# raulmur/ORB_SLAM

Measured on AMD Instinct MI355X. Metric: frames/s ORB extract+match @640x480, 1000 kp, higher is better.
Workload: dtype u8; 1 GPU; vga: 640x480 grayscale stream, 8 levels, nFeatures 1000, S-blocks frames, extract + Hamming top-2 match vs previous frame (BASELINE.json configs[1] + the frame-to-frame match of the metric); resident_frames_per_gpu=2048, lanes=4, parity_checked_frames=0, parity_mismatches=0, library_build_id=3635dfdd85252d64, lane_placement=2

## Files before the change

orb_slam_amd/csrc/k_fast.hip:

```cpp
#include <algorithm>
#include <type_traits>

#include "orbx_device.h"
#include "orbx_launch.h"
#include "k_blur_strip.h"

namespace orbx {

__device__ __forceinline__ int fast_pair_test(const uint8_t* c, int S, int v, int t) {
    const int x0 = c[3 * S], x1 = c[3 * S + 1], x2 = c[2 * S + 2], x3 = c[S + 3], x4 = c[3], x5 = c[-S + 3], x6 = c[-2 * S + 2], x7 = c[-3 * S + 1];
    const int x8 = c[-3 * S], x9 = c[-3 * S - 1], x10 = c[-2 * S - 2], x11 = c[-S - 3], x12 = c[-3], x13 = c[S - 3], x14 = c[2 * S - 2], x15 = c[3 * S - 1];
    const int a = imax3(imax3(imin(x0, x8), imin(x1, x9), imin(x2, x10)), imax3(imin(x3, x11), imin(x4, x12), imin(x5, x13)), imax(imin(x6, x14), imin(x7, x15)));
    const int bq = imin3(imin3(imax(x0, x8), imax(x1, x9), imax(x2, x10)), imin3(imax(x3, x11), imax(x4, x12), imax(x5, x13)), imin(imax(x6, x14), imax(x7, x15)));
    return (int)(v - a > t) | (int)(bq - v > t);
}

__device__ __forceinline__ int fast_score_raw(const uint8_t* c, int S, int v, int tmin) {
    int x[16];
    x[0] = c[3 * S]; x[1] = c[3 * S + 1]; x[2] = c[2 * S + 2]; x[3] = c[S + 3]; x[4] = c[3]; x[5] = c[-S + 3]; x[6] = c[-2 * S + 2]; x[7] = c[-3 * S + 1];
    x[8] = c[-3 * S]; x[9] = c[-3 * S - 1]; x[10] = c[-2 * S - 2]; x[11] = c[-S - 3]; x[12] = c[-3]; x[13] = c[S - 3]; x[14] = c[2 * S - 2]; x[15] = c[3 * S - 1];
    int hi3[16], lo3[16];
#pragma unroll
    for (int k = 0; k < 16; k++) {
        hi3[k] = imax3(x[k], x[(k + 1) & 15], x[(k + 2) & 15]);
// ... 16 lines not shown
struct FastHdr { int n_hi, n_lo, overflow, pad1; int wsum[8]; int pad2[4]; };
static_assert(sizeof(FastHdr) == 64, "LDS carve");

__device__ __forceinline__ int lane_rank(unsigned long long m) {
    return (int)__builtin_amdgcn_mbcnt_hi((unsigned)(m >> 32), __builtin_amdgcn_mbcnt_lo((unsigned)m, 0u));
}
struct CompassK { uint32_t R, KB, KD; };
__device__ __forceinline__ CompassK compass_consts(int t) {
    CompassK k;
    k.R = (uint32_t)compass_r(t) * 0x01010101u;
    k.KB = (uint32_t)compass_kb(t) * 0x01010101u;
    k.KD = (uint32_t)compass_kd(t) * 0x01010101u;
    return k;
}
__device__ __forceinline__ uint32_t compass4_dev(uint32_t C, uint32_t E, uint32_t W, uint32_t Nn, uint32_t Ss, const CompassK& k) {
    const uint32_t nc = ~C;
    const uint32_t hN = __builtin_amdgcn_lerp(Nn, nc, k.R), hS = __builtin_amdgcn_lerp(Ss, nc, k.R);
    const uint32_t hE = __builtin_amdgcn_lerp(E, nc, k.R), hW = __builtin_amdgcn_lerp(W, nc, k.R);
    const uint32_t br = (__builtin_amdgcn_lerp(hN, k.KB, 0u) | __builtin_amdgcn_lerp(hS, k.KB, 0u)) &
                        (__builtin_amdgcn_lerp(hE, k.KB, 0u) | __builtin_amdgcn_lerp(hW, k.KB, 0u));
    const uint32_t dN = __builtin_amdgcn_lerp(hN, k.KD, 0u), dS = __builtin_amdgcn_lerp(hS, k.KD, 0u);
    const uint32_t dE = __builtin_amdgcn_lerp(hE, k.KD, 0u), dW = __builtin_amdgcn_lerp(hW, k.KD, 0u);
    return (br | ~((dN & dS) | (dE & dW))) & 0x80808080u;
}
__global__ void k_eval_compass(const uint32_t* c, const uint32_t* e, const uint32_t* w, const uint32_t* nn, const uint32_t* ss, uint32_t* out, int n, int t) {
    const int i = blockIdx.x * blockDim.x + threadIdx.x;
    if (i < n) out[i] = compass4_dev(c[i], e[i], w[i], nn[i], ss[i], compass_consts(t));
}
int launch_eval_compass(const uint32_t* c, const uint32_t* e, const uint32_t* w, const uint32_t* nn, const uint32_t* ss, uint32_t* out, int n, int t) {
    hipLaunchKernelGGL(k_eval_compass, dim3((n + 255) / 256), dim3(256), 0, 0, c, e, w, nn, ss, out, n, t);
    return hipGetLastError() == hipSuccess ? ORBX_OK : ORBX_ERR_DEVICE;
}

template <bool ALIGNED, int NT, int PPT, bool GATHER = false>
__device__ __forceinline__ void fast_band_task(const Batch& b, int frame, int item, uint8_t* smem) {
    constexpr int NW = NT / 64;
    static_assert((NW & (NW - 1)) == 0, "wave roles rotate modulo NW");
    constexpr int Q0CAP = fast_q0cap(PPT), Q1CAP = FAST_Q1CAP, Q2CAP = FAST_Q2CAP, Q3CAP = FAST_Q3CAP;
    constexpr int WQ_BYTES = fast_wave_queue_bytes(PPT);
    const DevGeom& g = b.g;
    const BandGeom bg = b.bands[item];
    const int level = bg.level;
    const LevelGeom& L = g.lv[level];
    const int lane = threadIdx.x & 63, wave = ORBX_FAST_ROTATE ? (wave_id() + item) & (NW - 1) : wave_id(), tid = wave * 64 + lane;
    const int cw = bg.x1 - bg.x0 + 1, ch = bg.ey1 - bg.ey0 + 1;
    CellState* cst = b.cstate + (long long)frame * g.nbands_total + item;
    const int hint = b.fallback_hint ? (int)((uint32_t)cst->thr >> 8) : 0;
    if (cw <= 0 || ch <= 0) {
        if (tid == 0) { CellState st; st.n_all = 0; st.n_hi = 0; st.n_lo = 0; st.thr = g.tmin; *cst = st; }
        return;
    }
    const int own_lo = bg.y0 - bg.ey0, own_hi = bg.y1 - bg.ey0;
    const int gxb = (bg.x0 - 3) & ~3;
    const int xoff = (bg.x0 - 3) - gxb;
    const int nd = fast_row_dwords(xoff, cw);
    const int S = nd * 4;
    const int x_first = xoff + 3;
    const int nrows = ch + 6;
    FastHdr* hdr = reinterpret_cast<FastHdr*>(smem);
    unsigned long long* cmask = reinterpret_cast<unsigned long long*>(smem + sizeof(FastHdr));
    uint8_t* wq = smem + sizeof(FastHdr) + g.fast_max_chunks * 8 + wave * WQ_BYTES;
    uint32_t* q0 = reinterpret_cast<uint32_t*>(wq);
    uint16_t* q1 = reinterpret_cast<uint16_t*>(wq + Q0CAP * 4);
    uint16_t* q2 = q1 + Q1CAP;
    uint16_t* q3 = q2 + Q2CAP;
    uint8_t* s_img = smem + sizeof(FastHdr) + g.fast_max_chunks * 8 + NW * WQ_BYTES;
    uint8_t* s_sc = s_img + g.fast_max_img;
    const int q_own_lo = (3 + own_lo) * S, q_own_hi = (3 + own_hi + 1) * S;
    const int nchunks = (q_own_hi - q_own_lo + 63) >> 6;
    long long stride64;
    const uint8_t* src = plain_plane<GATHER>(b, L, level, frame, stride64);
    auto clear_lds = [&]() {
        for (int i = tid; i < ((nrows * S + 15) >> 4); i += NT) reinterpret_cast<uint4*>(s_sc)[i] = make_uint4(0, 0, 0, 0);
        if (tid < (int)(sizeof(FastHdr) / 4)) reinterpret_cast<int*>(hdr)[tid] = 0;
        for (int i = tid; i < nchunks; i += NT) cmask[i] = 0ull;
    };
    if (ALIGNED) {
        typedef const void __attribute__((address_space(1))) * gptr_t;
        typedef void __attribute__((address_space(3))) * lptr_t;
        const uint8_t* src0 = src + (long long)(bg.ey0 - 3) * stride64 + gxb;
        clear_lds();
        {
            const int cpr = nd >> 2, nchunks16 = nrows * cpr;
            const float inv_cpr = bg.inv_cpr;
            for (int q0 = 64 * wave; q0 < nchunks16; q0 += 64 * NW) {
                const int q = q0 + lane;
                int r, c;
                split_px(imin(q, nchunks16 - 1), cpr, inv_cpr, r, c);
                const uint8_t* ga = src0 + (long long)r * stride64 + 16 * c;
                if (q < nchunks16) __builtin_amdgcn_global_load_lds((gptr_t)ga, (lptr_t)(s_img + 16 * q0), 16, 0, 0);
            }
        }
        asm volatile("s_waitcnt vmcnt(0)" ::: "memory");
    } else {
        const int total = nrows * nd;
        const float inv_nd0 = bg.inv_nd;
        const uint8_t* src0 = src + (long long)(bg.ey0 - 3) * stride64 + gxb;
        const int xm = L.w - 1 - gxb;
        for (int i0 = 0; i0 < total; i0 += NT * 8) {
            uint32_t v4[8];
#pragma unroll
            for (int k = 0; k < 8; k++) {
                const int i = i0 + k * NT + tid;
                v4[k] = 0;
                if (i < total) {
                    int r, d;
                    split_px(i, nd, inv_nd0, r, d);
                    const uint8_t* row = src0 + (long long)r * stride64;
                    v4[k] = (uint32_t)row[imin(4 * d, xm)] | (uint32_t)row[imin(4 * d + 1, xm)] << 8 | (uint32_t)row[imin(4 * d + 2, xm)] << 16 |
                            (uint32_t)row[imin(4 * d + 3, xm)] << 24;
                }
            }
            if (i0 == 0) clear_lds();
#pragma unroll
            for (int k = 0; k < 8; k++) {
                const int i = i0 + k * NT + tid;
                if (i < total) reinterpret_cast<uint32_t*>(s_img)[i] = v4[k];
            }
        }
    }
    __syncthreads();

    constexpr int FAST_HINT_RUN = 6;
    int tmin = ORBX_FAST_TWO_PASS ? (hint >= FAST_HINT_RUN && g.fast_th > 7 ? 7 : g.fast_th) : g.tmin;
    const float inv_nd = bg.inv_nd;
    int n0 = 0, n1 = 0, n2 = 0, n3 = 0;

    auto score_vals = [&](bool on, int p) {
        int sc = 0;
        if (on) {
            const uint8_t* c = s_img + p;
            sc = fast_score_raw(c, S, c[0], tmin);
            s_sc[p] = (uint8_t)sc;
        }
        const unsigned long long mk = __ballot(sc != 0);
        if (mk) {
            const int add = __popcll(mk);
            if (n3 + add <= Q3CAP) { if (sc) q3[n3 + lane_rank(mk)] = (uint16_t)p; }
            n3 += add;
        }
    };
    auto score_step = [&](const uint16_t* q, int m) { score_vals(lane < m, lane < m ? (int)q[lane] : 0); };
    auto pair_step = [&](const uint16_t* q, int m) {
        int pass = 0, p = 0;
        if (lane < m) {
            p = q[lane];
            const uint8_t* c = s_img + p;
            pass = fast_pair_test(c, S, c[0], tmin);
        }
        const unsigned long long mk = __ballot(pass);
        if (mk) {
            if (pass) q2[n2 + lane_rank(mk)] = (uint16_t)p;
            n2 += __popcll(mk);
            if (n2 >= 64) { n2 -= 64; score_step(q2 + n2, 64); }
// ... 80 lines not shown
            if (s >= 7) atomicAdd(&hdr->n_lo, 1);
        }
    };
    if (!hdr->overflow) {
        int c_hi = 0, c_lo = 0;
        for (int i0 = 0; i0 < n3; i0 += 64) {
            const int i = i0 + lane;
            int s = 0;
            bool keep = false;
            if (i < n3) {
                const int p = q3[i];
                s = s_sc[p];
                keep = p >= q_own_lo && p < q_own_hi && nms_test(p, s);
            }
            c_hi += __popcll(__ballot(keep && s >= g.fast_th));
            c_lo += __popcll(__ballot(keep && s >= 7));
        }
        if (lane == 0 && (c_hi | c_lo)) { atomicAdd(&hdr->n_hi, c_hi); atomicAdd(&hdr->n_lo, c_lo); }
    } else {
        const int d_lo = q_own_lo >> 2, d_hi = q_own_hi >> 2;
        for (int i = d_lo + tid; i < d_hi; i += NT) {
            uint32_t sc4 = reinterpret_cast<const uint32_t*>(s_sc)[i];
            while (sc4) {
                const int j = (__ffs((int)sc4) - 1) >> 3;
                const int s = (int)((sc4 >> (8 * j)) & 255u);
                sc4 &= ~(255u << (8 * j));
                nms_px(4 * i + j, s);
            }
        }
    }
    __syncthreads();
    if (tmin <= 7 || __builtin_amdgcn_readfirstlane(hdr->n_hi) > 3) break;
    __syncthreads();
    clear_lds();
    tmin = 7;
    K = compass_consts(7);
    n0 = n1 = n2 = n3 = 0;
    __syncthreads();
    }
    Cand* out = b.cand + (long long)frame * g.frame_cands + L.cand_base + bg.cand_off;
    const float inv_S = bg.inv_s;
    int run_base = 0;
    for (int c0 = 0; c0 < nchunks; c0 += NT) {
        const bool busy = c0 + 64 * wave < nchunks;
        unsigned long long m = 0ull;
        int cnt = 0, incl = 0;
        if (busy) {
            if (c0 + tid < nchunks) m = cmask[c0 + tid];
            cnt = __popcll(m);
            incl = wave_scan_inclusive(cnt);
        }
        if (NW > 1) {
            if (lane == 63) hdr->wsum[wave] = incl;
            __syncthreads();
        }
        int run = run_base + incl - cnt, total = NW > 1 ? 0 : __builtin_amdgcn_readlane(incl, 63);
        if (NW > 1 && busy) {
#pragma unroll
            for (int wv = 0; wv < NW; wv++) { const int t = hdr->wsum[wv]; if (wv < wave) run += t; total += t; }
        }
        while (m) {
            const int bit = __ffsll((long long)m) - 1;
            m &= m - 1;
            const int p = q_own_lo + (c0 + tid) * 64 + bit;
            int r, xr;
            split_px(p, S, inv_S, r, xr);
            Cand e;
            e.pos = (uint32_t)(bg.x0 + xr - x_first) | ((uint32_t)(bg.ey0 + r - 3) << 16);
            e.resp = (float)s_sc[p];
            out[run++] = e;
        }
        run_base += total;
        if (NW > 1 && c0 + NT < nchunks) __syncthreads();
    }
    if (tid == 0) {
        CellState st;
        st.n_all = run_base; st.n_hi = hdr->n_hi; st.n_lo = hdr->n_lo;
        st.thr = tmin | ((st.n_hi <= 3 && g.fast_th > 7 ? imin(hint + 1, FAST_HINT_RUN) : 0) << 8);
        *cst = st;
    }
}

template <bool ALIGNED, int NT, int PPT, bool GATHER>
__device__ __forceinline__ void k_fast_cells_body(const Batch& b) {
    extern __shared__ __attribute__((aligned(16))) uint8_t smem[];
    int frame, item;
    if (!frame_item_magic(b, blockIdx.x, (unsigned)b.g.nbands_total, b.g.nbands_magic, frame, item)) return;
    fast_band_task<ALIGNED, NT, PPT, GATHER>(b, frame, item, smem);
}
template <bool ALIGNED, int NT, int PPT>
__global__ __launch_bounds__(NT) void k_fast_cells(Batch b) { k_fast_cells_body<ALIGNED, NT, PPT, false>(b); }
template <bool ALIGNED, int NT, int PPT>
__global__ __launch_bounds__(NT) void k_fast_cells_gather(Batch b) { k_fast_cells_body<ALIGNED, NT, PPT, true>(b); }

template <bool ALIGNED, bool SMALL, bool GATHER>
__device__ __forceinline__ void k_fast_blur_body(const Batch& b) {
    extern __shared__ __attribute__((aligned(16))) uint8_t smem[];
    constexpr FastShape A = SMALL ? FAST_SMALL : FAST_LARGE;
    constexpr int NW = A.threads / 64;
    const DevGeom& g = b.g;
    const int nblur = (g.nbtiles_total_s + NW - 1) / NW;
    const int per_frame = nblur + g.nbands_total;
    const int frame = blockIdx.x / per_frame, item = blockIdx.x - frame * per_frame;
    if (item < nblur) {
        const int t = item * NW + wave_id();
        if (t < g.nbtiles_total_s) blur_strip<ALIGNED, BLUR_ROWS_SMALL, GATHER>(b, frame, t);
    } else fast_band_task<ALIGNED, A.threads, A.ppt, GATHER>(b, frame, item - nblur, smem);
}
template <bool ALIGNED, bool SMALL>
__global__ __launch_bounds__(SMALL ? FAST_SMALL.threads : FAST_LARGE.threads) void k_fast_blur(Batch b) { k_fast_blur_body<ALIGNED, SMALL, false>(b); }
template <bool ALIGNED, bool SMALL>
__global__ __launch_bounds__(SMALL ? FAST_SMALL.threads : FAST_LARGE.threads) void k_fast_blur_gather(Batch b) { k_fast_blur_body<ALIGNED, SMALL, true>(b); }


int launch_fast(const Batch& b, const HostGeom& hg, hipStream_t stream, bool fuse_blur) {
    const DevGeom& g = hg.g;
    const int F = b.nframes;
    const bool aligned = (level0_bits(b) & 3) == 0;
    const size_t lds = (size_t)g.fast_lds_bytes;
    auto launch = [&](auto kern, int threads) -> bool {
        if (lds > 64 * 1024 && hipFuncSetAttribute(reinterpret_cast<const void*>(kern), hipFuncAttributeMaxDynamicSharedMemorySize, (int)lds) != hipSuccess) return false;
        hipLaunchKernelGGL(kern, dim3(frame_item_blocks(b, g.nbands_total)), dim3(threads), lds, stream, b);
        return true;
    };
    constexpr FastShape A = FAST_SMALL, B = FAST_LARGE;
    bool ok;
    if (fuse_blur) {
        const int threads = g.fast_small ? A.threads : B.threads;
        const int per_frame = (g.nbtiles_total_s + threads / 64 - 1) / (threads / 64) + g.nbands_total;
        auto launch2 = [&](auto kern) -> bool {
            if (lds > 64 * 1024 && hipFuncSetAttribute(reinterpret_cast<const void*>(kern), hipFuncAttributeMaxDynamicSharedMemorySize, (int)lds) != hipSuccess) return false;
            hipLaunchKernelGGL(kern, dim3(F * per_frame), dim3(threads), lds, stream, b);
            return true;
        };
        if (b.img_tab) {
            if (g.fast_small) ok = aligned ? launch2(k_fast_blur_gather<true, true>) : launch2(k_fast_blur_gather<false, true>);
            else ok = aligned ? launch2(k_fast_blur_gather<true, false>) : launch2(k_fast_blur_gather<false, false>);
        } else if (g.fast_small) ok = aligned ? launch2(k_fast_blur<true, true>) : launch2(k_fast_blur<false, true>);
        else ok = aligned ? launch2(k_fast_blur<true, false>) : launch2(k_fast_blur<false, false>);
    } else if (b.img_tab) {
        if (g.fast_small) ok = aligned ? launch(k_fast_cells_gather<true, A.threads, A.ppt>, A.threads) : launch(k_fast_cells_gather<false, A.threads, A.ppt>, A.threads);
        else ok = aligned ? launch(k_fast_cells_gather<true, B.threads, B.ppt>, B.threads) : launch(k_fast_cells_gather<false, B.threads, B.ppt>, B.threads);
    } else if (g.fast_small) ok = aligned ? launch(k_fast_cells<true, A.threads, A.ppt>, A.threads) : launch(k_fast_cells<false, A.threads, A.ppt>, A.threads);
    else ok = aligned ? launch(k_fast_cells<true, B.threads, B.ppt>, B.threads) : launch(k_fast_cells<false, B.threads, B.ppt>, B.threads);
    if (!ok) return ORBX_ERR_DEVICE;
    ORBX_LAUNCH_CHECK();
    return ORBX_OK;
}

}
```

orb_slam_amd/csrc/orbx_api.hip:

```cpp
#include <climits>
#include <cstdio>
#include <cstdlib>
#include <cstring>

#include "orbx_internal.h"

namespace orbx {
int launch_eval_math(int kind, const float* in0, const float* in1, float* out0, float* out1, int n);
int launch_eval_compass(const uint32_t* c, const uint32_t* e, const uint32_t* w, const uint32_t* nn, const uint32_t* ss, uint32_t* out, int n, int t);
int launch_eval_blur_window(const uint8_t* win, uint8_t* out, int n, int ties_even, int general);
void stage_timer_collect(StageTimer& t);
int launch_debug_nth(const float* d_resp, int n, int nth, int* d_out);
int launch_ingest(uint8_t* d_dst, const uint8_t* mapped_src, size_t bytes, hipStream_t stream);
}
using namespace orbx;

struct orbx_extractor {
    orbx_params p;
    std::string err;
    int gw = 0, gh = 0;
    HostGeom hg;
    struct __attribute__((visibility("hidden"))) Geom {
        DevBuf cells, cellrecs, bands, tabx, taby, pyr_tab;
        DevBuf pyr, blur, cand, sel, cstate, csel, cbands, level_total, level_count, status, long_cells;
    } geo;
    bool fallback_hint = true;
    DevBuf d_img1;
    PinnedBuf h_img1;
    DevBuf d_out1;
    PinnedBuf h_out1;
    bool zero_copy = true;
    Stream s1;
    int stop_after = -1;
    bool no_xcd_affinity = false;
    int od_min_frames = ORBX_OD_MIN_FRAMES_DEFAULT;
    int blur_on_demand = ORBX_BLUR_ON_DEMAND_DEFAULT;
    StageTimer timer;
    SideStream side;
    Batch last;
    bool have_last = false;
    int ph_done = 0;
    struct PhaseKey {
        const void *img, *kps, *desc, *n, *stream;
        int nframes, w, hgt, cap;
        ptrdiff_t row_stride, frame_stride;
        bool operator==(const PhaseKey& o) const {
            return img == o.img && kps == o.kps && desc == o.desc && n == o.n && stream == o.stream && nframes == o.nframes && w == o.w && hgt == o.hgt &&
                   cap == o.cap && row_stride == o.row_stride && frame_stride == o.frame_stride;
        }
    } ph_key = {};
    static constexpr int TAB_RING = 4;
    DevBuf d_tab;
    PinnedBuf h_tab;
    Event tab_ev[TAB_RING];
    int tab_next = 0;
    std::vector<ImgSrc> last_tab;
// ... 4 lines not shown
        Event up_ev[2], kern_ev[2];
        int next = 0;
    };
    HostUpload hup;
    HostUpload cup;
    DevBuf d_cring;
    PinnedBuf h_cimg1, h_gray1;
    DevBuf d_cimg1;
};

template <typename T>
static int upload(orbx_extractor* h, DevBuf& d, const std::vector<T>& v) {
    HIPCHK(h, d.ensure(std::max<size_t>(v.size(), 1) * sizeof(T)));
    if (!v.empty()) HIPCHK(h, hipMemcpy(d, v.data(), v.size() * sizeof(T), hipMemcpyHostToDevice));
    return ORBX_OK;
}

static int ensure_geometry(orbx_extractor* h, int w, int hgt) {
    if (h->gw == w && h->gh == hgt) return ORBX_OK;
    HIPCHK(h, hipDeviceSynchronize());
    h->geo = {};
    h->gw = h->gh = 0;
    h->have_last = false;
    HostGeom hg;
    int rc = build_geometry(h->p, w, hgt, hg, h->err);
    if (rc != ORBX_OK) return rc;
    h->hg = hg;
    const DevGeom& g = h->hg.g;
    const size_t B = (size_t)h->p.max_batch;
    orbx_extractor::Geom& d = h->geo;
    if ((rc = upload(h, d.cells, h->hg.cells)) != ORBX_OK) return rc;
    if ((rc = upload(h, d.cellrecs, h->hg.cellrecs)) != ORBX_OK) return rc;
    if ((rc = upload(h, d.bands, h->hg.bands)) != ORBX_OK) return rc;
    if ((rc = upload(h, d.tabx, h->hg.tabx)) != ORBX_OK) return rc;
    if ((rc = upload(h, d.taby, h->hg.taby)) != ORBX_OK) return rc;
    if ((rc = upload(h, d.pyr_tab, h->hg.pyr_tab)) != ORBX_OK) return rc;
    HIPCHK(h, d.pyr.ensure(B * g.frame_plane_bytes));
    HIPCHK(h, d.blur.ensure(B * g.frame_plane_bytes));
    HIPCHK(h, d.cand.ensure(B * std::max(g.frame_cands, 1) * sizeof(Cand)));
    HIPCHK(h, d.sel.ensure((B * std::max(g.frame_sel, 1) + 4) * sizeof(Cand)));
    HIPCHK(h, d.cstate.ensure(B * g.nbands_total * sizeof(CellState)));
    HIPCHK(h, hipMemset(d.cstate, 0, B * g.nbands_total * sizeof(CellState)));
    HIPCHK(h, d.csel.ensure(B * g.ncells_total * sizeof(CellSel)));
    HIPCHK(h, d.cbands.ensure(B * g.ncells_total * sizeof(CellBands)));
    HIPCHK(h, hipMemset(d.cbands, 0, B * g.ncells_total * sizeof(CellBands)));
    HIPCHK(h, d.level_total.ensure(B * MAX_LEVELS * sizeof(int32_t)));
    HIPCHK(h, d.level_count.ensure(B * MAX_LEVELS * sizeof(int32_t)));
    HIPCHK(h, hipMemset(d.level_total, 0, B * MAX_LEVELS * sizeof(int32_t)));
    HIPCHK(h, hipMemset(d.level_count, 0, B * MAX_LEVELS * sizeof(int32_t)));
    HIPCHK(h, d.status.ensure(B * sizeof(int32_t)));
    HIPCHK(h, d.long_cells.ensure((B * g.ncells_total + 64) * sizeof(int32_t)));
    HIPCHK(h, hipDeviceSynchronize());
    h->gw = w;
    h->gh = hgt;
    return ORBX_OK;
}

static void fill_batch(orbx_extractor* h, Batch& b) {
    const orbx_extractor::Geom& d = h->geo;
    b.g = h->hg.g; b.cells = d.cells.as<CellGeom>(); b.cellrec = d.cellrecs.as<CellRec>(); b.bands = d.bands.as<BandGeom>(); b.tabx = d.tabx.as<ResizeX>(); b.taby = d.taby.as<ResizeY>();
    b.pyr_tab = d.pyr_tab.as<int>(); b.pyr = d.pyr.as(); b.blur = d.blur.as();
    b.cand = d.cand.as<Cand>(); b.sel = d.sel.as<Cand>(); b.cstate = d.cstate.as<CellState>(); b.csel = d.csel.as<CellSel>(); b.cbands = d.cbands.as<CellBands>();
    b.level_total = d.level_total.as<int32_t>(); b.level_count = d.level_count.as<int32_t>(); b.status = d.status.as<int32_t>();
    b.long_cells = d.long_cells.as<int32_t>();
}

static void group_batch(orbx_extractor* h, Batch& b, int f0, int n, orbx_keypoint* d_kps, uint8_t* d_desc, int32_t* d_n, int cap, int32_t* d_status) {
    memset(&b, 0, sizeof(b));
    fill_batch(h, b);
    b.fallback_hint = h->fallback_hint ? 1 : 0;
    b.nframes = n;
    b.xcd_affinity = (b.nframes >= XCD_AFFINITY_MIN_FRAMES && !h->no_xcd_affinity) ? 1 : 0;
    b.blur_on_demand = h->blur_on_demand;
    b.od_min_frames = h->od_min_frames;
    b.out_kps = d_kps + (size_t)f0 * cap;
    b.out_desc = d_desc + (size_t)f0 * cap * 32;
    b.out_n = d_n + f0;
    b.out_status = d_status ? d_status + f0 : nullptr;
    b.cap = cap;
}

static hipMemoryType host_memory_type(const void* p) {
    hipPointerAttribute_t a;
    if (hipPointerGetAttributes(&a, p) != hipSuccess) {
        (void)hipGetLastError();
        return hipMemoryTypeUnregistered;
    }
    return a.type;
}

static int launch_group(orbx_extractor* h, const Batch& b, hipStream_t stream, int phases = ORBX_PHASE_ALL) {
    const int rc = launch_extract(b, h->hg, stream, h->stop_after, &h->timer, &h->side, phases);
    if (rc != ORBX_OK) { h->err = "kernel launch failed (no gfx950 code object for this device?)"; return rc; }
// ... 807 lines not shown
```

orb_slam_amd/csrc/orbx_geometry.hip:

```cpp
#include <cfloat>
#include <climits>
#include <cmath>
#include <cstdlib>
#include <cstring>

#include "k_resize_strip.h"
#include "orbx_internal.h"

namespace orbx {

static inline int round_even(double v) { return (int)std::lrint(v); }
static inline int floor_int(double v) { int i = (int)v; return i - (i > v); }
static inline int ceil_int(double v) { int i = (int)v; return i + (i < v); }
static inline int16_t sat16(float v) {
    int iv = round_even(v);
    return (int16_t)(iv < SHRT_MIN ? SHRT_MIN : iv > SHRT_MAX ? SHRT_MAX : iv);
}
static inline int align_up(int v, int a) { return (v + a - 1) / a * a; }

StripChoice resize_strip_choice(const HostGeom& hg, int level, long long src_stride, unsigned long long src_bits) {
    StripChoice sc = {0, 0};
    const DevGeom& g = hg.g;
    if (level < 1 || level >= g.nlevels) return sc;
    const LevelGeom& L = g.lv[level];
    const LevelGeom& P = g.lv[level - 1];
    if (!L.rz_window) return sc;
    long long stride = P.stride;
    if (level == 1) {
        stride = src_stride;
        if (((src_bits | (unsigned long long)stride) & 3) != 0 || stride < P.w) return sc;
    }
    const long long readable = rzs_readable(level == 1, stride, P.w);
    if (stride > RZS_LDS_BUDGET) return sc;
    const ResizeY* ty = hg.taby.data() + L.taby_off;
    sc.rows_out = rzs_pick_rows(ty, L.h, stride, readable);
    if (sc.rows_out) sc.lds_bytes = (int)rzs_lds_bytes(ty, L.h, sc.rows_out, stride, readable);
    return sc;
}

static int build_geometry_band(const orbx_params& p, int w, int h, HostGeom& out, std::string& err, const int band_px, const FastShape& shape) {
    const int threads = shape.threads;
    const int nl = p.nlevels;
    if (nl < 1 || nl > MAX_LEVELS) { err = "nlevels out of range [1,16]"; return ORBX_ERR_ARG; }
    if (p.nfeatures < 1) { err = "nfeatures must be >= 1"; return ORBX_ERR_ARG; }
    if (!(p.scale_factor > 1.0f) || p.scale_factor > 2.5f) { err = "scale_factor must be in (1, 2.5]"; return ORBX_ERR_ARG; }
    if (w < 1 || h < 1 || w > 16384 || h > 16384) { err = "image size out of range"; return ORBX_ERR_ARG; }
    if (p.score_type != ORBX_HARRIS_SCORE && p.score_type != ORBX_FAST_SCORE) { err = "score_type"; return ORBX_ERR_ARG; }

    out = HostGeom();
    DevGeom& g = out.g;
    memset(&g, 0, sizeof(g));
    g.nlevels = nl;
    g.score_type = p.score_type;
    g.fp_contract = p.fp_contract ? 1 : 0;
    g.fast_th = std::min(std::max(p.fast_th, 0), 255);
    g.tmin = std::min(g.fast_th, 7);

    const double scaleFactor = (double)p.scale_factor;
    out.scale.assign(nl, 1.f);
    out.inv_scale.assign(nl, 1.f);
    for (int i = 1; i < nl; i++) out.scale[i] = (float)(out.scale[i - 1] * scaleFactor);
    const float invScaleFactor = (float)(1.0f / scaleFactor);
    for (int i = 1; i < nl; i++) out.inv_scale[i] = out.inv_scale[i - 1] * invScaleFactor;
    out.features_per_level.assign(nl, 0);
    {
        const float factor = (float)(1.0 / scaleFactor);
        float per_scale = p.nfeatures * (1 - factor) / (1 - (float)std::pow((double)factor, (double)nl));
        int sum = 0;
        for (int l = 0; l < nl - 1; l++) {
            out.features_per_level[l] = round_even(per_scale);
// ... 88 lines not shown
                const bool skipX = (j == levelCols - 1) && (maxBX + 3 - (c.x0 - 3) <= 0);
                const bool skipY = (i == levelRows - 1) && (maxBY + 3 - (c.y0 - 3) <= 0);
                c.skipped = (skipX || skipY) ? 1 : 0;
                const int cw = std::max(0, c.x1 - c.x0 + 1), ch = std::max(0, c.y1 - c.y0 + 1);
                c.cand_off = cand_off;
                c.band0 = (int)out.bands.size();
                const int nb = std::max(1, (cw * ch + band_px - 1) / band_px);
                const int rb = std::max(1, (ch + nb - 1) / nb);
                c.nbands = 0;
                c.cand_cap = 0;
                for (int k = 0; k < nb; k++) {
                    BandGeom bg;
                    memset(&bg, 0, sizeof(bg));
                    bg.x0 = c.x0; bg.x1 = c.x1;
                    bg.y0 = (int16_t)(c.y0 + k * rb);
                    bg.y1 = (int16_t)std::min<int>(c.y1, bg.y0 + rb - 1);
                    if (k > 0 && bg.y0 > c.y1) break;
                    bg.ey0 = (int16_t)std::max<int>(c.y0, bg.y0 - 1);
                    bg.ey1 = (int16_t)std::min<int>(c.y1, bg.y1 + 1);
                    bg.level = l;
                    const int bh = std::max(0, bg.y1 - bg.y0 + 1);
                    bg.cand_off = cand_off;
                    bg.cand_cap = ((cw + 1) / 2) * ((bh + 1) / 2);
                    if (cw > 0) {
                        const int nd = fast_row_dwords((bg.x0 - 3) & 3, cw);
                        bg.inv_nd = 1.0f / (float)nd;
                        bg.inv_s = 1.0f / (float)(nd * 4);
                        bg.inv_cpr = 1.0f / (float)(nd >> 2);
                    }
                    cand_off += bg.cand_cap;
                    c.cand_cap += bg.cand_cap;
                    c.nbands++;
                    out.bands.push_back(bg);
                }
                out.cells.push_back(c);
            }
        for (int ci = L.cell_base; ci < L.cell_base + L.ncells; ci++) {
            const CellGeom& c = out.cells[ci];
            CellRec r;
            memset(&r, 0, sizeof(r));
            r.level = l; r.nbands = c.nbands; r.skipped = c.skipped; r.band0 = c.band0;
            r.sel_base = sel_base; r.plane_off = L.plane_off; r.stride = L.stride;
            r.cand_off = L.cand_base + c.cand_off;
            for (int k = 0; k < c.nbands && k < CELL_REC_BANDS; k++) r.band_cand[k] = L.cand_base + out.bands[c.band0 + k].cand_off;
            out.cellrecs.push_back(r);
        }
        cell_base += L.ncells;
        cand_base += cand_off;
        L.sel_base = sel_base;
        L.sel_cap = std::min(cand_off, L.ncells * L.nfeat_cell + L.ncells * L.ncells + L.ndesired + 64);
        sel_base += L.sel_cap;
        L.slot_base = slot_base;
        slot_base += L.ndesired;
        L.quad_base = quad_base;
        quad_base += (L.ndesired + 3) / 4;

        L.btiles_x = (L.w + 247) / 248;
        L.btiles_y = (L.h + BLUR_ROWS - 1) / BLUR_ROWS;
        L.btile_base = btile_base;
        btile_base += L.btiles_x * L.btiles_y;
        L.btiles_y_s = (L.h + BLUR_ROWS_SMALL - 1) / BLUR_ROWS_SMALL;
        L.btile_base_s = btile_base_s;
        btile_base_s += L.btiles_x * L.btiles_y_s;
        {
            const int nsteps = (L.h + 31) / 32;
            L.mb_strips = (L.w + 32 * MB_TILES - 1) / (32 * MB_TILES);
// ... 92 lines not shown
                        if (s0 < dk) src = is_x ? (out.tabx[Lk.tabx_off + s0].sx & ~3) : out.taby[Lk.taby_off + s0].sy0;
                        at(k - 1, i, 0) = src;
                    }
                    for (int i = 0; i < n; i++) {
                        const int e0 = std::min(at(k, i, 1), dk - 1);
                        int need = is_x ? out.tabx[Lk.tabx_off + e0].sx1 : out.taby[Lk.taby_off + e0].sy1;
                        need = std::max(need, at(k - 1, i + 1, 0) - 1);
                        if (is_x) need = std::min(need | 3, ds - 1);
                        at(k - 1, i, 1) = std::max(need, at(k - 1, i, 0));
                    }
                    at(k - 1, n, 1) = ds;
                }
                return base;
            };
            pg.xtab = chain(pg.ntx, tile[0], true, out.pyr_tab);
            pg.ytab = chain(pg.nty, tile[1], false, out.pyr_tab);
            int off = 0;
            for (int k = 0; k < pg.depth; k++) {
                int maxw = 4, maxh = 1;
                for (int i = 0; i < pg.ntx; i++) maxw = std::max(maxw, out.pyr_tab[pg.xtab + ((size_t)k * (pg.ntx + 1) + i) * 2 + 1] - out.pyr_tab[pg.xtab + ((size_t)k * (pg.ntx + 1) + i) * 2] + 1);
                for (int i = 0; i < pg.nty; i++) maxh = std::max(maxh, out.pyr_tab[pg.ytab + ((size_t)k * (pg.nty + 1) + i) * 2 + 1] - out.pyr_tab[pg.ytab + ((size_t)k * (pg.nty + 1) + i) * 2] + 1);
                pg.pitch[k] = align_up(maxw, 4) + 4;
                pg.lds_off[k] = off;
                off += align_up(pg.pitch[k] * maxh, 16);
            }
            pg.lds_bytes = off;
            if (off > 64 * 1024) { ok = false; break; }
            g.pyr[g.npyr_groups++] = pg;
            l0 += pg.depth;
        }
        if (!ok) { g.npyr_groups = 0; out.pyr_tab.clear(); }
    }
    {
        int max_px = 0, max_img = 0, max_chunks = 0;
        for (const BandGeom& c : out.bands) {
            const int cw = c.x1 - c.x0 + 1, ch = c.ey1 - c.ey0 + 1;
            if (cw <= 0 || ch <= 0) continue;
            max_px = std::max(max_px, cw * ch);
            if (cw > shape.max_cw) { err = "grid cell wider than " + std::to_string(shape.max_cw) + " pixels"; return ORBX_ERR_CAPACITY; }
            const int nd = fast_row_dwords(3, cw);
            max_img = std::max(max_img, nd * 4 * (ch + 6));
            max_chunks = std::max(max_chunks, (nd * 4 * (c.y1 - c.y0 + 1) + 63) / 64);
        }
        if (max_px > 65535 || max_img > 65536) { err = "grid cell band larger than 64 KiB with its halo"; return ORBX_ERR_CAPACITY; }
        g.fast_max_img = align_up(std::max(max_img, 16), 16);
        g.fast_max_chunks = align_up(max_chunks + 1, 2);
        g.fast_lds_bytes = 64  + g.fast_max_chunks * 8 + (threads / 64) * fast_wave_queue_bytes(shape.ppt) + 2 * g.fast_max_img + 16;
        if (g.fast_lds_bytes > 160 * 1024) { err = "grid cell does not fit the 160 KiB LDS"; return ORBX_ERR_CAPACITY; }
    }
    {
        int max_cell = 1, max_level = 1;
        for (const CellGeom& c : out.cells) max_cell = std::max(max_cell, (int)c.cand_cap);
        for (int l = 0; l < nl; l++) max_level = std::max(max_level, g.lv[l].sel_cap);
        g.sel_lds_entries = std::min(std::max(max_cell, max_level), 2048);
        g.sel_lds_cell = align_up(g.sel_lds_entries * ((int)sizeof(Cand) + 4), 16);
        g.sel_lds_level = g.sel_lds_cell;
        if (g.sel_lds_cell > 160 * 1024 || g.sel_lds_level > 160 * 1024) { err = "keypoint list does not fit the 160 KiB LDS"; return ORBX_ERR_CAPACITY; }
    }
    for (int l = 0; l < MAX_LEVELS; l++) {
        const bool live = l < nl;
        g.cell_bases[l] = live ? g.lv[l].cell_base : INT_MAX;
        g.quad_bases[l] = live ? g.lv[l].quad_base : INT_MAX;
        g.btile_bases[l] = live ? g.lv[l].btile_base : INT_MAX;
        g.btile_bases_s[l] = live ? g.lv[l].btile_base_s : INT_MAX;
        g.mb_bases[l] = live ? g.lv[l].mb_base : INT_MAX;
    }
    g.ncells_total = cell_base;
    g.nbands_total = (int)out.bands.size();
    g.nbands_magic = g.nbands_total > 1 ? (uint32_t)((1ull << 32) / (unsigned)g.nbands_total) + 1u : 0u;
    g.nbtiles_total = btile_base;
    g.nbtiles_total_s = btile_base_s;
    g.nmb_total = mb_base;
    g.nslots = slot_base;
    g.nquads = quad_base;
    g.frame_plane_bytes = align_up(plane_off, 256);
    g.frame_cands = cand_base;
    g.frame_sel = sel_base;
    return ORBX_OK;
// ... 42 lines not shown
```

orb_slam_amd/csrc/orbx_internal.h:

```cpp
#pragma once
#include <hip/hip_runtime.h>
#include <stdint.h>
#include <string>
#include <vector>

#include "orbx.h"
#include "orbx_host.h"

namespace orbx {

constexpr int MAX_LEVELS = 16;
constexpr int EDGE = 16;
constexpr int HALF_PATCH = 15;

struct Cand {
    uint32_t pos;
    float resp;
};

struct ResizeX { int16_t sx, sx1, a0, a1; };
struct ResizeY { int16_t sy0, sy1, b0, b1; };

struct LevelGeom {
    int w, h;
// ... 68 lines not shown
#endif
constexpr int MB_WAVES = ORBX_MB_WAVES;
constexpr int BLUR_ROWS = ORBX_BLUR_ROWS;
constexpr int BLUR_ROWS_SMALL = 8;
constexpr int RZ_ROWS = ORBX_RZ_ROWS;
struct FastShape { int threads, ppt, band_px, max_cw; };
#ifndef ORBX_FS
#define ORBX_FS 256, 1, 8192, 500
#endif
#ifndef ORBX_FL
#define ORBX_FL 256, 2, 7168, 6500
#endif
constexpr FastShape FAST_SMALL = {ORBX_FS};
constexpr FastShape FAST_LARGE = {ORBX_FL};
#ifndef ORBX_FAST_TWO_PASS
#define ORBX_FAST_TWO_PASS 1
#endif
#ifndef ORBX_FAST_ROTATE
#define ORBX_FAST_ROTATE 1
#endif
constexpr int FAST_Q1CAP = 192, FAST_Q2CAP = 128, FAST_Q3CAP = 192;
constexpr int fast_q0cap(int) { return 128; }
constexpr int fast_wave_queue_bytes(int ppt) { return fast_q0cap(ppt) * 4 + FAST_Q1CAP * 2 + FAST_Q2CAP * 2 + FAST_Q3CAP * 2; }
__host__ __device__ constexpr int fast_row_dwords(int xoff, int cw) { return (((xoff + cw + 6 + 3) >> 2) + 3) & ~3; }
struct BandGeom {
    int16_t x0, x1;
    int16_t y0, y1;
    int16_t ey0, ey1;
    int32_t level;
    int32_t cand_off;
    int32_t cand_cap;
    float inv_nd, inv_s, inv_cpr;
};

constexpr int XCD_AFFINITY_MIN_FRAMES = 64;
#ifndef ORBX_PYR_DEPTH
#define ORBX_PYR_DEPTH 4, 4
#endif
constexpr int PYR_MAX_GROUPS = 4, PYR_MAX_DEPTH = 8;
struct PyrGroup {
    int l0, depth;
    int ntx, nty;
    int xtab, ytab;
    int lds_off[PYR_MAX_DEPTH];
    int pitch[PYR_MAX_DEPTH];
    int lds_bytes;
};
#ifndef ORBX_PYR_TILE
#define ORBX_PYR_TILE 16, 16
#endif

constexpr int QUOTA_LDS_PER_CELL = 10;
constexpr int QUOTA_MAX_CELLS = 160 * 1024 / QUOTA_LDS_PER_CELL / 64 * 64;
struct CellState { int32_t n_all, n_hi, n_lo, thr; };
constexpr int CELL_REC_BANDS = 8;
struct alignas(64) CellRec {
    int32_t level, nbands, skipped, band0;
    int32_t sel_base;
    int32_t plane_off, stride;
    int32_t cand_off;
    int32_t band_cand[CELL_REC_BANDS];
};
struct alignas(16) CellSel { int32_t n_all, thr, nretain, out_off; };
struct alignas(32) CellBands { int32_t n[CELL_REC_BANDS]; };
static_assert(sizeof(CellRec) == 64 && sizeof(CellSel) == 16 && sizeof(CellBands) == 32, "one scalar load per record");

// ... 4 lines not shown
    uint32_t nbands_magic;
    int nbtiles_total, nbtiles_total_s;
    int nmb_total;
    int nslots;
    int nquads;
    int quota_cells;
    int score_type, fast_th, tmin;
    int fp_contract;
    int frame_plane_bytes;
    int frame_cands;
    int frame_sel;
    int sel_lds_cell, sel_lds_level, sel_lds_entries;
    int fast_max_img, fast_max_chunks, fast_lds_bytes;
    int fast_threads;
    int fast_small;
    int npyr_groups;
    PyrGroup pyr[PYR_MAX_GROUPS];
    int umax[HALF_PATCH + 1];
    int cell_bases[MAX_LEVELS], quad_bases[MAX_LEVELS], btile_bases[MAX_LEVELS], btile_bases_s[MAX_LEVELS], mb_bases[MAX_LEVELS];
    LevelGeom lv[MAX_LEVELS];
};

struct ImgSrc {
    const uint8_t* data;
    long long row_stride;
};
static_assert(sizeof(ImgSrc) == 16, "one scalar dwordx4 per table entry");

struct Batch {
    DevGeom g;
    const CellGeom* cells;
    const CellRec* cellrec;
    const BandGeom* bands;
    const ResizeX* tabx;
    const ResizeY* taby;
    const int* pyr_tab;
    const uint8_t* img;
    long long img_row_stride, img_frame_stride;
    uint8_t* pyr;
    uint8_t* blur;
    Cand* cand;
    Cand* sel;
    CellState* cstate;
    int fallback_hint;
    CellSel* csel;
    CellBands* cbands;
    int32_t* level_total;
    int32_t* level_count;
    int32_t* status;
    int32_t* long_cells;
    orbx_keypoint* out_kps;
    uint8_t* out_desc;
    int32_t* out_n;
    int32_t* out_status;
    int cap;
    int nframes;
    int xcd_affinity;
    int od_min_frames;
    int blur_on_demand;
    const ImgSrc* img_tab;
    unsigned long long img_tab_bits;
    long long img_tab_min_stride;
    long long img_tab_max_stride;
};

static inline unsigned long long level0_bits(const Batch& b) {
    return b.img_tab ? b.img_tab_bits : ((uintptr_t)b.img | (unsigned long long)b.img_row_stride | (unsigned long long)b.img_frame_stride);
}
static inline long long level0_min_stride(const Batch& b) { return b.img_tab ? b.img_tab_min_stride : b.img_row_stride; }
static inline long long level0_max_stride(const Batch& b) { return b.img_tab ? b.img_tab_max_stride : b.img_row_stride; }

struct ColorArgs {
    const uint8_t* src;
    long long src_row_stride, src_frame_stride;
    const ImgSrc* tab;
    unsigned long long tab_bits;
    uint8_t* dst;
    uint8_t* dst2;
    long long dst_row_stride, dst_frame_stride;
    int w, h;
    int f0;
    int cpr, items;
};
static inline int pix_channels(int fmt) {
    switch (fmt) {
        case ORBX_PIX_GRAY8: return 1;
        case ORBX_PIX_RGB8: case ORBX_PIX_BGR8: return 3;
        case ORBX_PIX_RGBA8: case ORBX_PIX_BGRA8: return 4;
        default: return 0;
    }
}
int launch_to_gray(const ColorArgs& a, int nframes, int fmt, hipStream_t stream);

struct HostGeom {
    DevGeom g;
    std::vector<CellGeom> cells;
    std::vector<CellRec> cellrecs;
    std::vector<BandGeom> bands;
    std::vector<ResizeX> tabx;
    std::vector<ResizeY> taby;
    std::vector<int> pyr_tab;
    std::vector<int> features_per_level;
    std::vector<float> scale, inv_scale;
};

int build_geometry(const orbx_params& p, int w, int h, HostGeom& out, std::string& err);

struct StripChoice { int rows_out, lds_bytes; };
StripChoice resize_strip_choice(const HostGeom& hg, int level, long long src_stride, unsigned long long src_bits);
int resize_form(const Batch& b, const HostGeom& hg, int level, StripChoice& sc);

enum Stage { ST_PYRAMID = 0, ST_FAST_CELLS, ST_QUOTA, ST_CELL_SELECT, ST_LEVEL_SELECT, ST_BLUR, ST_DESCRIBE, ST_COUNT };

struct StageTimer {
    bool enabled = false;
    std::vector<hipEvent_t> pool;
    std::vector<int> pool_stage;
    double ms[ST_COUNT] = {0};
    long launches[ST_COUNT] = {0};
};

struct SideStream {
    Stream aux;
    Event fork, join;
};
int launch_extract(const Batch& b, const HostGeom& hg, hipStream_t stream, int stop_after, StageTimer* timer, const SideStream* side,
                   int phases = ORBX_PHASE_ALL);
bool describe_od_supported(const Batch& b, const HostGeom& hg);
int launch_describe_od(const Batch& b, const HostGeom& hg, hipStream_t stream);

}
// ... 1 lines not shown
```

Baseline: 501,700 frames/s.

## Precompute per-band FAST records on host and load them as one scalar record

Adds a 64-byte BandRec per band, built on the host, that holds the derived geometry (gxb, S, nrows, chunk counts, own-row offsets, source offset, candidate base). The FAST kernel loads it as a single scalar-constant read instead of recomputing the values from BandGeom and LevelGeom. Address math drops to 24-bit multiplies with a 32-bit offset, which the host now guards with a pitch check. The previous-threshold hint load is moved so it overlaps the image-to-LDS copy. This trims scalar prologue work and memory latency per band block, at the cost of another device table and new size limits that can reject launches.

```diff
diff --git a/orb_slam_amd/csrc/k_fast.hip b/orb_slam_amd/csrc/k_fast.hip
--- a/orb_slam_amd/csrc/k_fast.hip
+++ b/orb_slam_amd/csrc/k_fast.hip
@@ -72,6 +72,15 @@
     return hipGetLastError() == hipSuccess ? ORBX_OK : ORBX_ERR_DEVICE;
 }
 
+template <bool GATHER>
+__device__ __forceinline__ void fast_name_args(const Batch& b) {
+    const DevGeom& g = b.g;
+    asm volatile("" ::"s"(b.xcd_affinity), "s"(b.nframes), "s"(g.nbands_total), "s"(g.nbands_magic), "s"(b.bandrec), "s"(b.cstate), "s"(b.fallback_hint),
+                 "s"(g.fast_max_chunks), "s"(g.fast_max_img), "s"(b.pyr), "s"(g.frame_plane_bytes));
+    if constexpr (GATHER) asm volatile("" ::"s"(b.img_tab));
+    else asm volatile("" ::"s"(b.img), "s"(b.img_row_stride), "s"(b.img_frame_stride));
+}
+
 template <bool ALIGNED, int NT, int PPT, bool GATHER = false>
 __device__ __forceinline__ void fast_band_task(const Batch& b, int frame, int item, uint8_t* smem) {
     constexpr int NW = NT / 64;
@@ -79,24 +88,13 @@
     constexpr int Q0CAP = fast_q0cap(PPT), Q1CAP = FAST_Q1CAP, Q2CAP = FAST_Q2CAP, Q3CAP = FAST_Q3CAP;
     constexpr int WQ_BYTES = fast_wave_queue_bytes(PPT);
     const DevGeom& g = b.g;
-    const BandGeom bg = b.bands[item];
-    const int level = bg.level;
-    const LevelGeom& L = g.lv[level];
+    typedef const rec16_t __attribute__((address_space(4)))* c16_t;
+    typedef const rec4_t __attribute__((address_space(4)))* c4_t;
+    rec16_t vrec = *((c16_t)(uintptr_t)b.bandrec + item);
+    rec4_t vsrc = {0, 0, 0, 0};
+    if constexpr (GATHER) vsrc = *((c4_t)(uintptr_t)b.img_tab + frame);
     const int lane = threadIdx.x & 63, wave = ORBX_FAST_ROTATE ? (wave_id() + item) & (NW - 1) : wave_id(), tid = wave * 64 + lane;
-    const int cw = bg.x1 - bg.x0 + 1, ch = bg.ey1 - bg.ey0 + 1;
     CellState* cst = b.cstate + (long long)frame * g.nbands_total + item;
-    const int hint = b.fallback_hint ? (int)((uint32_t)cst->thr >> 8) : 0;
-    if (cw <= 0 || ch <= 0) {
-        if (tid == 0) { CellState st; st.n_all = 0; st.n_hi = 0; st.n_lo = 0; st.thr = g.tmin; *cst = st; }
-        return;
-    }
-    const int own_lo = bg.y0 - bg.ey0, own_hi = bg.y1 - bg.ey0;
-    const int gxb = (bg.x0 - 3) & ~3;
-    const int xoff = (bg.x0 - 3) - gxb;
-    const int nd = fast_row_dwords(xoff, cw);
-    const int S = nd * 4;
-    const int x_first = xoff + 3;
-    const int nrows = ch + 6;
     FastHdr* hdr = reinterpret_cast<FastHdr*>(smem);
     unsigned long long* cmask = reinterpret_cast<unsigned long long*>(smem + sizeof(FastHdr));
     uint8_t* wq = smem + sizeof(FastHdr) + g.fast_max_chunks * 8 + wave * WQ_BYTES;
@@ -106,37 +104,62 @@
     uint16_t* q3 = q2 + Q2CAP;
     uint8_t* s_img = smem + sizeof(FastHdr) + g.fast_max_chunks * 8 + NW * WQ_BYTES;
     uint8_t* s_sc = s_img + g.fast_max_img;
-    const int q_own_lo = (3 + own_lo) * S, q_own_hi = (3 + own_hi + 1) * S;
-    const int nchunks = (q_own_hi - q_own_lo + 63) >> 6;
-    long long stride64;
-    const uint8_t* src = plain_plane<GATHER>(b, L, level, frame, stride64);
-    auto clear_lds = [&]() {
-        for (int i = tid; i < ((nrows * S + 15) >> 4); i += NT) reinterpret_cast<uint4*>(s_sc)[i] = make_uint4(0, 0, 0, 0);
+    auto clear_lds = [&](int n16, int nmask) {
+        for (int i = tid; i < n16; i += NT) reinterpret_cast<uint4*>(s_sc)[i] = make_uint4(0, 0, 0, 0);
         if (tid < (int)(sizeof(FastHdr) / 4)) reinterpret_cast<int*>(hdr)[tid] = 0;
-        for (int i = tid; i < nchunks; i += NT) cmask[i] = 0ull;
-    };
+        for (int i = tid; i < nmask; i += NT) cmask[i] = 0ull;
+    };
+    if constexpr (GATHER) asm volatile("" : "+s"(vrec), "+s"(vsrc));
+    else asm volatile("" : "+s"(vrec));
+    const BandRec bg = __builtin_bit_cast(BandRec, vrec);
+    const int level = bg.level;
+    const int cw = bg.x1 - bg.x0 + 1, ch = bg.ey1 - bg.ey0 + 1;
+    if (cw <= 0 || ch <= 0) {
+        if (tid == 0) { CellState st; st.n_all = 0; st.n_hi = 0; st.n_lo = 0; st.thr = g.tmin; *cst = st; }
+        return;
+    }
+    const int gxb = bg.gxb;
+    const int S = bg.S, nd = S >> 2;
+    const int x_first = bg.x0 - gxb;
+    const int nrows = bg.nrows, nchunks16 = bg.nchunks16;
+    const int q_own_lo = bg.q_own_lo, q_own_hi = bg.q_own_hi;
+    const int nchunks = bg.nchunks;
+    const uint8_t* src0;
+    unsigned stride;
+    if (level == 0) {
+        const uint8_t* base;
+        long long stride64;
+        if constexpr (GATHER) { const ImgSrc e = __builtin_bit_cast(ImgSrc, vsrc); base = e.data; stride64 = e.row_stride; }
+        else { base = b.img + (long long)frame * b.img_frame_stride; stride64 = b.img_row_stride; }
+        src0 = base + (long long)(bg.ey0 - 3) * stride64 + gxb;
+        stride = (unsigned)stride64;
+    } else {
+        src0 = b.pyr + (long long)frame * g.frame_plane_bytes + bg.src_off;
+        stride = (unsigned)bg.stride;
+    }
+    typedef const int __attribute__((address_space(4)))* cint_t;
+    int thr_prev = 0;
     if (ALIGNED) {
         typedef const void __attribute__((address_space(1))) * gptr_t;
         typedef void __attribute__((address_space(3))) * lptr_t;
-        const uint8_t* src0 = src + (long long)(bg.ey0 - 3) * stride64 + gxb;
-        clear_lds();
+        clear_lds(nchunks16, nchunks);
         {
-            const int cpr = nd >> 2, nchunks16 = nrows * cpr;
+            const int cpr = S >> 4;
             const float inv_cpr = bg.inv_cpr;
             for (int q0 = 64 * wave; q0 < nchunks16; q0 += 64 * NW) {
                 const int q = q0 + lane;
                 int r, c;
                 split_px(imin(q, nchunks16 - 1), cpr, inv_cpr, r, c);
-                const uint8_t* ga = src0 + (long long)r * stride64 + 16 * c;
-                if (q < nchunks16) __builtin_amdgcn_global_load_lds((gptr_t)ga, (lptr_t)(s_img + 16 * q0), 16, 0, 0);
-            }
-        }
+                const unsigned off = __umul24((unsigned)r, stride) + 16u * (unsigned)c;
+                if (q < nchunks16) __builtin_amdgcn_global_load_lds((gptr_t)(src0 + off), (lptr_t)(s_img + 16 * q0), 16, 0, 0);
+            }
+        }
+        if (b.fallback_hint) thr_prev = *(cint_t)(uintptr_t)&cst->thr;
         asm volatile("s_waitcnt vmcnt(0)" ::: "memory");
     } else {
         const int total = nrows * nd;
         const float inv_nd0 = bg.inv_nd;
-        const uint8_t* src0 = src + (long long)(bg.ey0 - 3) * stride64 + gxb;
-        const int xm = L.w - 1 - gxb;
+        const int xm = bg.xm;
         for (int i0 = 0; i0 < total; i0 += NT * 8) {
             uint32_t v4[8];
 #pragma unroll
@@ -146,20 +169,23 @@
                 if (i < total) {
                     int r, d;
                     split_px(i, nd, inv_nd0, r, d);
-                    const uint8_t* row = src0 + (long long)r * stride64;
+                    const uint8_t* row = src0 + __umul24((unsigned)r, stride);
                     v4[k] = (uint32_t)row[imin(4 * d, xm)] | (uint32_t)row[imin(4 * d + 1, xm)] << 8 | (uint32_t)row[imin(4 * d + 2, xm)] << 16 |
                             (uint32_t)row[imin(4 * d + 3, xm)] << 24;
                 }
             }
-            if (i0 == 0) clear_lds();
+            if (i0 == 0) clear_lds(nchunks16, nchunks);
 #pragma unroll
             for (int k = 0; k < 8; k++) {
                 const int i = i0 + k * NT + tid;
                 if (i < total) reinterpret_cast<uint32_t*>(s_img)[i] = v4[k];
             }
         }
+        if (b.fallback_hint) thr_prev = *(cint_t)(uintptr_t)&cst->thr;
     }
     __syncthreads();
+    asm volatile("" : "+s"(thr_prev));
+    const int hint = (int)((uint32_t)thr_prev >> 8);
 
     constexpr int FAST_HINT_RUN = 6;
     int tmin = ORBX_FAST_TWO_PASS ? (hint >= FAST_HINT_RUN && g.fast_th > 7 ? 7 : g.fast_th) : g.tmin;
@@ -306,13 +332,13 @@
     __syncthreads();
     if (tmin <= 7 || __builtin_amdgcn_readfirstlane(hdr->n_hi) > 3) break;
     __syncthreads();
-    clear_lds();
+    clear_lds(nchunks16, nchunks);
     tmin = 7;
     K = compass_consts(7);
     n0 = n1 = n2 = n3 = 0;
     __syncthreads();
     }
-    Cand* out = b.cand + (long long)frame * g.frame_cands + L.cand_base + bg.cand_off;
+    Cand* out = b.cand + (long long)frame * g.frame_cands + bg.cand;
     const float inv_S = bg.inv_s;
     int run_base = 0;
     for (int c0 = 0; c0 < nchunks; c0 += NT) {
@@ -358,6 +384,7 @@
 template <bool ALIGNED, int NT, int PPT, bool GATHER>
 __device__ __forceinline__ void k_fast_cells_body(const Batch& b) {
     extern __shared__ __attribute__((aligned(16))) uint8_t smem[];
+    fast_name_args<GATHER>(b);
     int frame, item;
     if (!frame_item_magic(b, blockIdx.x, (unsigned)b.g.nbands_total, b.g.nbands_magic, frame, item)) return;
     fast_band_task<ALIGNED, NT, PPT, GATHER>(b, frame, item, smem);
@@ -373,6 +400,7 @@
     constexpr FastShape A = SMALL ? FAST_SMALL : FAST_LARGE;
     constexpr int NW = A.threads / 64;
     const DevGeom& g = b.g;
+    fast_name_args<GATHER>(b);
     const int nblur = (g.nbtiles_total_s + NW - 1) / NW;
     const int per_frame = nblur + g.nbands_total;
     const int frame = blockIdx.x / per_frame, item = blockIdx.x - frame * per_frame;
@@ -392,6 +420,8 @@
     const int F = b.nframes;
     const bool aligned = (level0_bits(b) & 3) == 0;
     const size_t lds = (size_t)g.fast_lds_bytes;
+    const long long pitch = std::max<long long>(level0_max_stride(b), g.lv[0].stride);
+    if (pitch >= (1ll << 24) || (long long)hg.fast_max_rows * pitch + 65536 >= (1ll << 32)) return ORBX_ERR_ARG;
     auto launch = [&](auto kern, int threads) -> bool {
         if (lds > 64 * 1024 && hipFuncSetAttribute(reinterpret_cast<const void*>(kern), hipFuncAttributeMaxDynamicSharedMemorySize, (int)lds) != hipSuccess) return false;
         hipLaunchKernelGGL(kern, dim3(frame_item_blocks(b, g.nbands_total)), dim3(threads), lds, stream, b);
diff --git a/orb_slam_amd/csrc/orbx_api.hip b/orb_slam_amd/csrc/orbx_api.hip
--- a/orb_slam_amd/csrc/orbx_api.hip
+++ b/orb_slam_amd/csrc/orbx_api.hip
@@ -21,7 +21,7 @@
     int gw = 0, gh = 0;
     HostGeom hg;
     struct __attribute__((visibility("hidden"))) Geom {
-        DevBuf cells, cellrecs, bands, tabx, taby, pyr_tab;
+        DevBuf cells, cellrecs, bands, bandrecs, tabx, taby, pyr_tab;
         DevBuf pyr, blur, cand, sel, cstate, csel, cbands, level_total, level_count, status, long_cells;
     } geo;
     bool fallback_hint = true;
@@ -92,6 +92,7 @@
     if ((rc = upload(h, d.cells, h->hg.cells)) != ORBX_OK) return rc;
     if ((rc = upload(h, d.cellrecs, h->hg.cellrecs)) != ORBX_OK) return rc;
     if ((rc = upload(h, d.bands, h->hg.bands)) != ORBX_OK) return rc;
+    if ((rc = upload(h, d.bandrecs, h->hg.bandrecs)) != ORBX_OK) return rc;
     if ((rc = upload(h, d.tabx, h->hg.tabx)) != ORBX_OK) return rc;
     if ((rc = upload(h, d.taby, h->hg.taby)) != ORBX_OK) return rc;
     if ((rc = upload(h, d.pyr_tab, h->hg.pyr_tab)) != ORBX_OK) return rc;
@@ -118,7 +119,7 @@
 
 static void fill_batch(orbx_extractor* h, Batch& b) {
     const orbx_extractor::Geom& d = h->geo;
-    b.g = h->hg.g; b.cells = d.cells.as<CellGeom>(); b.cellrec = d.cellrecs.as<CellRec>(); b.bands = d.bands.as<BandGeom>(); b.tabx = d.tabx.as<ResizeX>(); b.taby = d.taby.as<ResizeY>();
+    b.g = h->hg.g; b.cells = d.cells.as<CellGeom>(); b.cellrec = d.cellrecs.as<CellRec>(); b.bands = d.bands.as<BandGeom>(); b.bandrec = d.bandrecs.as<BandRec>(); b.tabx = d.tabx.as<ResizeX>(); b.taby = d.taby.as<ResizeY>();
     b.pyr_tab = d.pyr_tab.as<int>(); b.pyr = d.pyr.as(); b.blur = d.blur.as();
     b.cand = d.cand.as<Cand>(); b.sel = d.sel.as<Cand>(); b.cstate = d.cstate.as<CellState>(); b.csel = d.csel.as<CellSel>(); b.cbands = d.cbands.as<CellBands>();
     b.level_total = d.level_total.as<int32_t>(); b.level_count = d.level_count.as<int32_t>(); b.status = d.status.as<int32_t>();
diff --git a/orb_slam_amd/csrc/orbx_geometry.hip b/orb_slam_amd/csrc/orbx_geometry.hip
--- a/orb_slam_amd/csrc/orbx_geometry.hip
+++ b/orb_slam_amd/csrc/orbx_geometry.hip
@@ -36,6 +36,30 @@
     sc.rows_out = rzs_pick_rows(ty, L.h, stride, readable);
     if (sc.rows_out) sc.lds_bytes = (int)rzs_lds_bytes(ty, L.h, sc.rows_out, stride, readable);
     return sc;
+}
+
+static BandRec make_band_rec(const BandGeom& bg, const LevelGeom& L, int level) {
+    BandRec r;
+    memset(&r, 0, sizeof(r));
+    r.x0 = bg.x0; r.x1 = bg.x1; r.y0 = bg.y0; r.y1 = bg.y1; r.ey0 = bg.ey0; r.ey1 = bg.ey1;
+    r.level = level;
+    r.cand_cap = bg.cand_cap;
+    r.cand = L.cand_base + bg.cand_off;
+    r.stride = L.stride; r.plane_off = L.plane_off;
+    r.inv_nd = bg.inv_nd; r.inv_s = bg.inv_s; r.inv_cpr = bg.inv_cpr;
+    const int cw = bg.x1 - bg.x0 + 1, ch = bg.ey1 - bg.ey0 + 1;
+    if (cw <= 0 || ch <= 0) return r;
+    const int gxb = (bg.x0 - 3) & ~3, xoff = (bg.x0 - 3) - gxb;
+    const int nd = fast_row_dwords(xoff, cw), S = nd * 4, nrows = ch + 6;
+    r.gxb = (int16_t)gxb;
+    r.xm = (int16_t)(L.w - 1 - gxb);
+    r.S = (uint16_t)S; r.nrows = (uint16_t)nrows;
+    r.nchunks16 = (uint16_t)(nrows * (nd >> 2));
+    const int q_own_lo = (3 + bg.y0 - bg.ey0) * S, q_own_hi = (3 + bg.y1 - bg.ey0 + 1) * S;
+    r.q_own_lo = (uint16_t)q_own_lo; r.q_own_hi = (uint16_t)q_own_hi;
+    r.nchunks = (uint16_t)((q_own_hi - q_own_lo + 63) >> 6);
+    if (level > 0) r.src_off = L.plane_off + (bg.ey0 - 3) * L.stride + gxb;
+    return r;
 }
 
 static int build_geometry_band(const orbx_params& p, int w, int h, HostGeom& out, std::string& err, const int band_px, const FastShape& shape) {
@@ -190,6 +214,7 @@
                     c.cand_cap += bg.cand_cap;
                     c.nbands++;
                     out.bands.push_back(bg);
+                    out.bandrecs.push_back(make_band_rec(bg, L, l));
                 }
                 out.cells.push_back(c);
             }
@@ -348,7 +373,7 @@
         if (!ok) { g.npyr_groups = 0; out.pyr_tab.clear(); }
     }
     {
-        int max_px = 0, max_img = 0, max_chunks = 0;
+        int max_px = 0, max_img = 0, max_chunks = 0, max_rows = 0;
         for (const BandGeom& c : out.bands) {
             const int cw = c.x1 - c.x0 + 1, ch = c.ey1 - c.ey0 + 1;
             if (cw <= 0 || ch <= 0) continue;
@@ -356,10 +381,12 @@
             if (cw > shape.max_cw) { err = "grid cell wider than " + std::to_string(shape.max_cw) + " pixels"; return ORBX_ERR_CAPACITY; }
             const int nd = fast_row_dwords(3, cw);
             max_img = std::max(max_img, nd * 4 * (ch + 6));
+            max_rows = std::max(max_rows, ch + 6);
             max_chunks = std::max(max_chunks, (nd * 4 * (c.y1 - c.y0 + 1) + 63) / 64);
         }
         if (max_px > 65535 || max_img > 65536) { err = "grid cell band larger than 64 KiB with its halo"; return ORBX_ERR_CAPACITY; }
         g.fast_max_img = align_up(std::max(max_img, 16), 16);
+        out.fast_max_rows = max_rows;
         g.fast_max_chunks = align_up(max_chunks + 1, 2);
         g.fast_lds_bytes = 64  + g.fast_max_chunks * 8 + (threads / 64) * fast_wave_queue_bytes(shape.ppt) + 2 * g.fast_max_img + 16;
         if (g.fast_lds_bytes > 160 * 1024) { err = "grid cell does not fit the 160 KiB LDS"; return ORBX_ERR_CAPACITY; }
diff --git a/orb_slam_amd/csrc/orbx_internal.h b/orb_slam_amd/csrc/orbx_internal.h
--- a/orb_slam_amd/csrc/orbx_internal.h
+++ b/orb_slam_amd/csrc/orbx_internal.h
@@ -124,6 +124,20 @@
     int32_t cand_cap;
     float inv_nd, inv_s, inv_cpr;
 };
+struct alignas(64) BandRec {
+    int16_t x0, x1, y0, y1, ey0, ey1;
+    int32_t level;
+    int32_t cand_cap;
+    int32_t cand;
+    int32_t stride, plane_off;
+    int32_t src_off;
+    int16_t gxb, xm;
+    uint16_t S, nrows;
+    uint16_t nchunks16, nchunks;
+    uint16_t q_own_lo, q_own_hi;
+    float inv_nd, inv_s, inv_cpr;
+};
+static_assert(sizeof(BandRec) == 64, "one scalar load per record");
 
 constexpr int XCD_AFFINITY_MIN_FRAMES = 64;
 #ifndef ORBX_PYR_DEPTH
@@ -194,6 +208,7 @@
     const CellGeom* cells;
     const CellRec* cellrec;
     const BandGeom* bands;
+    const BandRec* bandrec;
     const ResizeX* tabx;
     const ResizeY* taby;
     const int* pyr_tab;
@@ -259,6 +274,8 @@
     std::vector<CellGeom> cells;
     std::vector<CellRec> cellrecs;
     std::vector<BandGeom> bands;
+    std::vector<BandRec> bandrecs;
+    int fast_max_rows = 0;
     std::vector<ResizeX> tabx;
     std::vector<ResizeY> taby;
     std::vector<int> pyr_tab;
```

Result: no change. 505,700 frames/s, median of 6 (+0.8%).
